# Nishad-Sharma/gpuRaytracer

Hardware: AMD Instinct MI355X
Metric: Msamples/sec (pixels×spp) Cornell box 1080p at 1/2/4/8 MI355X; HBM GB/s (higher is better)
Workload: dtype f32; 1 GPU; cornell_1920x1080_256spp_b3; width=1920, height=1080, spp_per_gpu=256, spp_frame=256, bounces=3, parallelism=single GPU

## Files before the change

gpuraytracer_amd/_native.py:

```python
from __future__ import annotations

import ctypes
import os

ABI_VERSION = 11
_HERE = os.path.dirname(os.path.abspath(__file__))
library_path = os.environ.get("RTPT_LIB") or os.path.join(_HERE, "librtpt.so")


class float3(ctypes.Structure):

    _fields_ = [("x", ctypes.c_float), ("y", ctypes.c_float), ("z", ctypes.c_float),
                ("_pad", ctypes.c_float)]

    def __iter__(self):
        return iter((self.x, self.y, self.z))


class float4(ctypes.Structure):
    _fields_ = [("x", ctypes.c_float), ("y", ctypes.c_float), ("z", ctypes.c_float),
                ("w", ctypes.c_float)]


class int2(ctypes.Structure):
# ... 235 lines not shown
                                               ctypes.POINTER(MaterialGPU),
                                               ctypes.POINTER(float3),
                                               ctypes.POINTER(SquareLightGPU),
                                               ctypes.POINTER(ctypes.c_uint32),
                                               ctypes.POINTER(SphereGPU)]),
    "rt_render_mis": (ctypes.c_int, [_P, ctypes.POINTER(MisParamsC), _P, _P]),
    "rt_scene_cornell_box_mis": (ctypes.c_int, [ctypes.c_int32, ctypes.c_int32,
                                                ctypes.POINTER(CameraGPU),
                                                ctypes.POINTER(MaterialGPU),
                                                ctypes.POINTER(float3),
                                                ctypes.POINTER(SquareLightGPU),
                                                ctypes.POINTER(ctypes.c_uint32)]),
    "rt_tonemap_rgba8": (None, [_P, ctypes.c_size_t, _P]),
    "rt_scene_describe": (ctypes.c_int, [ctypes.POINTER(SceneDesc), ctypes.POINTER(SceneInfo)]),
    "rt_scene_describe_ex": (ctypes.c_int, [ctypes.POINTER(SceneDesc), ctypes.POINTER(CreateOptions),
                                            ctypes.POINTER(SceneInfo)]),
    "rt_debug_camera_candidates": (ctypes.c_int, [ctypes.POINTER(SceneDesc)] + [ctypes.c_int32] * 4 + [_P]),
    "rt_debug_shadow_candidates": (ctypes.c_int, [ctypes.POINTER(SceneDesc)] + [ctypes.c_int32] * 4 +
                                   [_P, ctypes.POINTER(ctypes.c_int32)]),
    "rt_debug_cluster_kinds": (ctypes.c_int, [ctypes.POINTER(SceneDesc), ctypes.POINTER(ctypes.c_uint32),
                                              ctypes.c_uint32, ctypes.POINTER(ctypes.c_uint32)]),
    "rt_debug_light_mask": (ctypes.c_int, [ctypes.POINTER(SceneDesc), ctypes.POINTER(ctypes.c_uint64), _P,
                                           ctypes.c_uint32]),
}


class RtError(RuntimeError):

    def __init__(self, status: int, message: str):
        super().__init__(f"{STATUS.get(status, status)}: {message}")
        self.status = status


def _preload_hip_runtime():
    if os.environ.get("RTPT_SYSTEM_HIP") == "1":
        return
    import importlib.util
    spec = importlib.util.find_spec("torch")
    if spec is None or not spec.submodule_search_locations:
        return
    for d in spec.submodule_search_locations:
        cand = os.path.join(d, "lib", "libamdhip64.so")
        if os.path.exists(cand):
            ctypes.CDLL(cand, mode=ctypes.RTLD_GLOBAL)
            return

# ... 31 lines not shown
```

gpuraytracer_amd/csrc/rt_api.cpp:

```cpp
#include <rccl/rccl.h>

#include <stdio.h>
#include <stdlib.h>
#include <string.h>

#include <chrono>
#include <new>
#include <vector>

#include "rt_api_internal.hpp"

using namespace rtapi;

namespace {

class DevBuf {
public:
    DevBuf() = default;
    DevBuf(DevBuf&& o) noexcept : p_(o.p_), bytes_(o.bytes_) { o.p_ = nullptr; o.bytes_ = 0; }
    DevBuf& operator=(DevBuf&& o) noexcept {
        std::swap(p_, o.p_);
        std::swap(bytes_, o.bytes_);
        return *this;
    }
// ... 45 lines not shown
    kTriIsect, kTriShade, kPairIsect, kClusters, kSphLds, kSphLdsId,
    kSphBox,
    kSphIsect, kSphShade, kSphNodes, kSphPerm, kMisShade, kSceneArrays
};

}

struct rt_ctx {
    int device = 0;
    Stream stream;
    Event ev0, ev1;
    Event ev_u0, ev_u1;
    Event ev_tiles;
    rt::CompiledScene scene;
    DevBuf d_scene[kSceneArrays];
    DevBuf d_tri_nodes;
    uint32_t tri_build = kDefaultTriBuild;
    DevBuf d_tri_sorted, d_tri_perm;
    DevBuf d_refit;
    uint32_t tri_bvh_nodes = 0;
    rt::SceneTables tab{};
    bool sph_compact = false;
    uint64_t light_mask = 0;
    uint32_t tri_bvh_build_used = 0;
    uint32_t tri_leaf_max = 1;
    float tri_bvh_build_ms = 0.0f;
    size_t tri_bvh_temp_bytes = 0;
    float scene_compile_ms = 0.0f;
    DevBuf d_mis_tab;
    uint32_t mis_tab_S = 0;
    DevBuf d_mis_part;
    DevBuf d_out, d_out8;
    DevBuf d_rays, d_hits;
    DevBuf d_aov[3];
    DevBuf d_den[6];
    DevBuf d_seeds;
    bool seeds_ready = false;
    uint32_t seed_max = 0xFFFFFFFFu;
    DevBuf d_sum;
    bool sum_valid = false;
    uint32_t sum_row_start = 0, sum_row_step = 0, sum_row_count = 0;
    uint32_t sum_first = 0, sum_samples = 0;
    bool timed = false;
    rt::LaunchInfo launch{};
    bool launched = false;
    ncclComm_t comm = nullptr;
// ... 269 lines not shown
    const uint64_t total = (uint64_t)(p->accumulate ? c->sum_samples : 0u) + p->spp;
    if (total == 0 || total > 0xFFFFFFFFull)
        return fail(c, RT_ERR_INVALID_ARG, "samples in the sum must be in [1, 2^32)");

    const size_t pixels = (size_t)count * (size_t)c->scene.cam.W;
    int st;
    if ((st = check_out_format(c, p->flags)) != RT_OK) return st;
    const size_t out_bytes = pixels * pixel_bytes(p->flags);
    if (sums) {
        if (c->d_sum.bytes() < pixels * sizeof(float4)) c->sum_valid = false;
        if ((st = reserve(c, c->d_sum, pixels * sizeof(float4), "hipMalloc(sum)")) != RT_OK) return st;
    }
    void* kout = want_out ? out : nullptr;
    if (want_out && !out_is_device) {
        if ((st = reserve(c, c->d_out, out_bytes, "hipMalloc(out staging)")) != RT_OK) return st;
        kout = c->d_out.as<void>();
    }

    rt::KParams K;
    memset(&K, 0, sizeof(K));
    set_tables(&K, c->tab);
    K.tri_shade = c->d_scene[kTriShade].as<float4>();
    K.light_mask = c->light_mask;
    K.sph_lds = c->sph_compact ? c->d_scene[kSphLds].as<uint32_t>() : nullptr;
    K.sph_lds_id = c->d_scene[kSphLdsId].as<uint16_t>();
    K.sph_shade = c->d_scene[kSphShade].as<float4>();
    K.seeds = c->d_seeds.as<uint32_t>();
    K.sum = sums ? c->d_sum.as<float4>() : nullptr;
    K.out = kout;
    K.nE = c->scene.sph_lds_entries;
    set_camera(&K, c->scene.cam);
    memcpy(K.light_center, c->scene.light.center, sizeof(K.light_center));
    {
        uint32_t by, bz;
        memcpy(&by, &K.light_center[1], 4);
        memcpy(&bz, &K.light_center[2], 4);
        K.light_plain = (by != 0x80000000u && bz != 0x80000000u) ? 1u : 0u;
    }
    memcpy(K.light_color, c->scene.light.color, sizeof(K.light_color));
    K.spp = p->spp;
    K.sample_base = p->sample_base;
    K.row_start = start;
    K.row_step = step;
    K.row_count = count;
    K.accumulate = p->accumulate ? 1u : 0u;
    K.samples_total = (uint32_t)total;
// ... 413 lines not shown
    if (!compile_desc(d, ro.build, &c->scene, &err)) {
        delete c;
        return fail(nullptr, RT_ERR_INVALID_ARG, err);
    }
    c->scene_compile_ms = std::chrono::duration<float, std::milli>(clk::now() - t_compile).count();
    int status = RT_OK;
    std::string msg;
    do {
        if ((e = hipStreamCreateWithFlags(&c->stream.h, hipStreamNonBlocking)) != hipSuccess) {
            status = RT_ERR_NO_DEVICE; msg = std::string("hipStreamCreate: ") + hipGetErrorString(e); break;
        }
        if ((e = hipEventCreate(&c->ev0.h)) != hipSuccess || (e = hipEventCreate(&c->ev1.h)) != hipSuccess ||
            (e = hipEventCreateWithFlags(&c->ev_tiles.h, hipEventDisableTiming)) != hipSuccess) {
            status = RT_ERR_NO_DEVICE; msg = std::string("hipEventCreate: ") + hipGetErrorString(e); break;
        }
        if ((e = upload_scene(c)) != hipSuccess) {
            status = RT_ERR_OUT_OF_MEMORY; msg = std::string("scene upload: ") + hipGetErrorString(e); break;
        }
        if (needs_tri_bvh(c) && (status = build_tri_bvh(c, &msg)) != RT_OK) break;
        const size_t npx = (size_t)c->scene.cam.W * (size_t)c->scene.cam.H;
        if ((e = c->d_seeds.reserve(npx * sizeof(uint32_t))) != hipSuccess) {
            status = RT_ERR_OUT_OF_MEMORY; msg = std::string("hipMalloc(seeds): ") + hipGetErrorString(e); break;
        }
    } while (0);
    if (status != RT_OK) {
        delete c;
        return fail(nullptr, status, msg);
    }
    finish_scene(c);
    *out_ctx = c;
    return RT_OK;
}

int rt_destroy(rt_ctx* c) {
    if (!c) return RT_OK;
    DeviceGuard g(c->device);
    delete c;
    return RT_OK;
}

int rt_update_scene(rt_ctx* c, const rt_scene_desc* d, uint32_t flags) {
    static_assert(sizeof(rt_update_stats) == 32, "rt_update_stats layout");
    if (!c) return fail(nullptr, RT_ERR_INVALID_ARG, "ctx is null");
    if (!d) return fail(c, RT_ERR_INVALID_ARG, "rt_update_scene: scene is null");
    if (!d->camera) return fail(c, RT_ERR_INVALID_ARG, "rt_update_scene: camera is null");
    if (!d->square_lights || d->n_square_lights < 1)
// ... 251 lines not shown
int rt_debug_tri_bvh(const rt_ctx* c, rt_tri_bvh_dump* dump) {
    if (!c || !dump) return fail(nullptr, RT_ERR_INVALID_ARG, "null argument");
    if (!c->broken.empty()) return fail(const_cast<rt_ctx*>(c), RT_ERR_STATE, c->broken);
    if (!c->tri_bvh_build_used || !c->d_tri_nodes) return RT_ERR_STATE;
    const size_t nT = c->scene.tri_isect.size(), nn = c->tri_bvh_nodes;
    dump->n_triangles = (uint32_t)nT;
    dump->nodes_per_layout = (uint32_t)nn;
    dump->leaf_max = c->tri_leaf_max;
    dump->margin = c->scene.margin;
    DeviceGuard g(c->device);
    const struct { void* dst; const DevBuf& src; size_t bytes; } copies[4] = {
        {dump->nodes, c->d_tri_nodes, rt::kTriCompactLayouts * nn * sizeof(uint4)},
        {dump->sorted, c->d_tri_sorted, nT * sizeof(rt::TriIsect)},
        {dump->perm, c->d_tri_perm, nT * sizeof(uint32_t)},
        {dump->isect, c->d_scene[kTriIsect], nT * sizeof(rt::TriIsect)}};
    for (const auto& cp : copies) {
        if (!cp.dst) continue;
        const hipError_t e = hipMemcpy(cp.dst, cp.src.as<void>(), cp.bytes, hipMemcpyDeviceToHost);
        if (e != hipSuccess) return RT_ERR_LAUNCH;
    }
    return RT_OK;
}

int rt_last_launch(const rt_ctx* c, rt_launch_info* info) {
    if (!c || !info) return fail(nullptr, RT_ERR_INVALID_ARG, "null argument");
    if (!c->launched) return RT_ERR_STATE;
    memset(info, 0, sizeof(*info));
    static_assert(sizeof(info->kernel) == sizeof(c->launch.kernel), "kernel name buffer");
    memcpy(info->kernel, c->launch.kernel, sizeof(info->kernel));
    info->kernel[sizeof(info->kernel) - 1] = 0;
    info->lanes_per_pixel = c->launch.lanes;
    info->halton_tables = c->launch.tables;
    info->small_index = c->launch.small;
    info->block_threads = c->launch.threads;
    info->grid_x = c->launch.grid_x;
    info->grid_y = c->launch.grid_y;
    info->lds_bytes = c->launch.lds;
    return RT_OK;
}

int rt_debug_stats(rt_ctx* c, uint64_t* out, int n) {
    if (!c || !out || n <= 0) return fail(c, RT_ERR_INVALID_ARG, "null argument");
    DeviceGuard g(c->device);
    hipError_t e = rt::read_debug_stats(reinterpret_cast<unsigned long long*>(out), n);
    if (e == hipErrorNotSupported) return fail(c, RT_ERR_STATE, "not an RT_STATS build");
    if (e != hipSuccess) return hip_fail(c, RT_ERR_LAUNCH, "read stats", e);
// ... 10 lines not shown
```

gpuraytracer_amd/csrc/rt_api_host.cpp:

```cpp
#include <string.h>

#include <thread>
#include <vector>

#include "rt_api_internal.hpp"
#include "rt_beam.hpp"
#include "rt_mathcheck.hpp"
#include "rt_shaft.hpp"

namespace rtapi {

bool resolve_options(const rt_create_options* o, Resolved* r, const char** why) {
    *r = Resolved();
    if (!o) return true;
    for (uint32_t v : o->reserved)
        if (v != 0) { *why = "rt_create_options.reserved must be zero"; return false; }
    switch (o->scene_layout) {
        case RT_LAYOUT_AUTO: r->mem = rt::SceneMem::kAuto; break;
        case RT_LAYOUT_PAIRS: r->mem = rt::SceneMem::kPairLds; break;
        case RT_LAYOUT_SINGLE: r->mem = rt::SceneMem::kLdsSingle; break;
        case RT_LAYOUT_GLOBAL: r->mem = rt::SceneMem::kSmem; break;
        case RT_LAYOUT_PAIRS_SMEM: r->mem = rt::SceneMem::kPairSmem; break;
        case RT_LAYOUT_SORTED: r->mem = rt::SceneMem::kPairSorted; break;
        case RT_LAYOUT_BVH: r->mem = rt::SceneMem::kTriBvh; break;
        default: *why = "rt_create_options.scene_layout out of range"; return false;
    }
    if (o->lanes_per_pixel != 0 && o->lanes_per_pixel != 1 && o->lanes_per_pixel != 4 &&
        o->lanes_per_pixel != 16) {
        *why = "rt_create_options.lanes_per_pixel must be 0, 1, 4 or 16";
// ... 278 lines not shown
int rt_debug_cluster_kinds(const rt_scene_desc* d, uint32_t* flags, uint32_t capacity, uint32_t* n_clusters) {
    if (!desc_ok(d) || !n_clusters || (!flags && capacity)) return fail(nullptr, RT_ERR_INVALID_ARG, "null argument");
    rt::CompiledScene s;
    const char* err = nullptr;
    if (!compile_desc(d, rt::BuildOptions(), &s, &err)) return fail(nullptr, RT_ERR_INVALID_ARG, err);
    const size_t rec = 4 * rt::kCluF4, nC = s.clusters.size() / rec;
    *n_clusters = (uint32_t)nC;
    for (size_t c = 0; c < nC && c < capacity; ++c) memcpy(&flags[c], &s.clusters[c * rec + 15], 4);
    return RT_OK;
}

int rt_debug_light_mask(const rt_scene_desc* d, uint64_t* mask, float* records, uint32_t capacity_triangles) {
    if (!desc_ok(d) || !mask || (!records && capacity_triangles))
        return fail(nullptr, RT_ERR_INVALID_ARG, "null argument");
    rt::CompiledScene s;
    const char* err = nullptr;
    if (!compile_desc(d, rt::BuildOptions(), &s, &err)) return fail(nullptr, RT_ERR_INVALID_ARG, err);
    *mask = rt::light_mask(s);
    for (size_t k = 0; k < s.tri_shade.size() && k < capacity_triangles; ++k)
        memcpy(records + 16 * k, s.tri_shade[k].s, sizeof(s.tri_shade[k].s));
    return RT_OK;
}

int rt_debug_tri_bvh_host(const rt_scene_desc* d, const rt_create_options* opt, rt_tri_bvh_dump* dump) {
    if (!desc_ok(d) || !dump) return fail(nullptr, RT_ERR_INVALID_ARG, "null argument");
    Resolved ro;
    const char* why = nullptr;
    if (!resolve_options(opt, &ro, &why)) return fail(nullptr, RT_ERR_INVALID_ARG, why);
    rt::CompiledScene s;
    const char* err = nullptr;
    if (!compile_desc(d, ro.build, &s, &err)) return fail(nullptr, RT_ERR_INVALID_ARG, err);
    const size_t nT = s.tri_isect.size();
    dump->n_triangles = (uint32_t)nT;
    dump->nodes_per_layout = 0;
    dump->leaf_max = tri_leaf_clamp(ro.tri_leaf_max);
    dump->margin = s.margin;
    if (nT == 0) return fail(nullptr, RT_ERR_INVALID_ARG, "the scene has no triangles");
    if (dump->isect) memcpy(dump->isect, s.tri_isect.data(), nT * sizeof(rt::TriIsect));
    if (!dump->nodes && !dump->sorted && !dump->perm) return RT_OK;
    HostTree t;
    if (!rt::build_tri_sah(s.tri_isect, s.margin, &t.nodes, &t.sorted, &t.perm, ro.tri_leaf_max, ro.tri_leaf_cost))
        return fail(nullptr, RT_ERR_INVALID_ARG, "triangle BVH build: too many triangles (2^24)");
    dump_host_tree(t, dump);
    return RT_OK;
}

// ... 155 lines not shown
```

gpuraytracer_amd/csrc/rt_halton.hpp:

```cpp
#pragma once
#include <hip/hip_runtime.h>

#include "rt_kernel.hpp"

namespace rt {
namespace {

constexpr uint32_t kPrimes[24] = RT_PRIMES_INIT;

template <uint32_t D>
__device__ __forceinline__ float halton(uint32_t i) {
    static_assert(D < 24, "Halton dimension outside primes[]");
    constexpr uint32_t b = kPrimes[D];
    constexpr float invB = 1.0f / (float)b;
    float f = 1.0f;
    float r = 0.0f;
    while (i > 0) {
        f = f * invB;
        r = r + f * (float)(i % b);
        i = i / b;
    }
    return r;
}

// ... 39 lines not shown
#pragma unroll
        for (int k = 0; k < nd; ++k) {
            f = f * invB;
            float digit;
            x = digit_step<b>(x, digit);
            r = r + f * digit;
        }
        return r;
    }
}

constexpr int kTabDigits[24] = {0, 6, 4, 3, 2, 2, 0, 2, 2, 2, 2, 0, 0, 0, 0, 0, 0, 0, 0, 0, 0, 0, 0, 0};
constexpr uint32_t ipow(uint32_t b, int k) { return k == 0 ? 1u : b * ipow(b, k - 1); }
constexpr uint32_t tab_size(int D) { return kTabDigits[D] ? ipow(kPrimes[D], kTabDigits[D]) : 0u; }
constexpr uint32_t tab_offset(int D) { return D == 0 ? 0u : tab_offset(D - 1) + tab_size(D - 1); }
constexpr uint32_t kHaltonTabFloats = tab_offset(24);
constexpr float f_after(uint32_t b, int k) {
    float f = 1.0f;
    for (int j = 0; j < k; ++j) f = f * (1.0f / (float)b);
    return f;
}

template <uint32_t D>
__device__ __forceinline__ void fill_halton_table(float* tab, uint32_t tid, uint32_t nthreads) {
    constexpr uint32_t b = kPrimes[D];
    constexpr int k = kTabDigits[D];
    constexpr float invB = 1.0f / (float)b;
    constexpr uint32_t off = tab_offset(D), size = tab_size(D);
    for (uint32_t v0 = tid; v0 < size; v0 += nthreads) {
        uint32_t v = v0;
        float f = 1.0f;
        float r = 0.0f;
#pragma unroll
        for (int j = 0; j < k; ++j) {
            f = f * invB;
            r = r + f * (float)(v % b);
            v = v / b;
        }
        tab[off + v0] = r;
    }
}

__device__ __forceinline__ void fill_halton_tables(float* tab, uint32_t tid, uint32_t nthreads) {
    fill_halton_table<1>(tab, tid, nthreads);
    fill_halton_table<2>(tab, tid, nthreads);
    fill_halton_table<3>(tab, tid, nthreads);
    fill_halton_table<4>(tab, tid, nthreads);
    fill_halton_table<5>(tab, tid, nthreads);
    fill_halton_table<7>(tab, tid, nthreads);
    fill_halton_table<8>(tab, tid, nthreads);
    fill_halton_table<9>(tab, tid, nthreads);
    fill_halton_table<10>(tab, tid, nthreads);
    static_assert(kHaltonTabFloats == 729 + 625 + 343 + 121 + 169 + 361 + 529 + 841 + 961,
                  "table list");
}

template <uint32_t D>
__device__ __forceinline__ float halton_tab(uint32_t i, const float* tab) {
    constexpr uint32_t b = kPrimes[D];
    constexpr int k = kTabDigits[D];
    constexpr int nd = halton_digits(b, kSmallIndexMax);
    constexpr float invB = 1.0f / (float)b;
    constexpr uint32_t bk = ipow(b, k), off = tab_offset(D);
    static_assert(k > 0 && k < nd, "dimension without a table");
    float low;
    float x = digit_step<bk>((float)i, low);
    float r = tab[off + (uint32_t)low];
    constexpr float fk = f_after(b, k);
    float f = fk;
#pragma unroll
    for (int j = k; j < nd; ++j) {
        f = f * invB;
        float digit;
        x = digit_step<b>(x, digit);
        r = r + f * digit;
    }
    return r;
// ... 13 lines not shown
```

gpuraytracer_amd/csrc/rt_kernel.hip:

```cpp
#include <hip/hip_runtime.h>
#include <hip/hip_fp16.h>

#include <stddef.h>
#include <stdio.h>
#ifdef RT_LDS_CHECK
#include <hsa/hsa.h>
#endif

#include "rt_kernel.hpp"
#include "rt_halton.hpp"
#include "rt_beam.hpp"
#include "rt_shaft.hpp"
#include "rt_pixel.hpp"
#include "rt_trace.hpp"

namespace rt {

#ifdef RT_LDS_CHECK
__device__ uint32_t g_lds_overflow;
__device__ __forceinline__ bool lds_short(size_t end) {
    const uint32_t grp = ((const uint32_t*)__builtin_amdgcn_dispatch_ptr())[7];
    const size_t dyn = grp - __builtin_amdgcn_groupstaticsize();
    if (end <= dyn) return false;
    if (threadIdx.x == 0) atomicMax(&g_lds_overflow, (uint32_t)end);
// ... 423 lines not shown
#define RT_TRI_WAVES 8
#endif
__global__ __launch_bounds__(block_threads(GEO),
                             SPH ? kMinWavesPerEuSph
                                 : (GEO == kGeoPairClu ? kMinWavesPerEuClu
                                                       : (GEO == kGeoTriBvh ? RT_TRI_WAVES : kMinWavesPerEu)))
void path_trace_kernel(KParams P) {
    constexpr uint32_t NT = block_threads(GEO), WR = waves_per_row(GEO), WC = waves_per_col(GEO);
    extern __shared__ float4 lds[];
    SceneView sv;
    const SceneTables T = tables_of(P);
    if (geo_staged(GEO)) {
        const StagedF4<uint32_t> n = staged_f4(GEO, T.nT, T.nP, T.nC);
        RT_LDS_GUARD(16 * (size_t)(n.rec + n.clu) + (GEO == kGeoPairClu ? 4 * (size_t)kHaltonTabFloats : 0));
        stage_records<GEO, NT>(lds, T);
        if (GEO == kGeoSphLds) {
            __shared__ float sph_stash[GEO == kGeoSphLds ? 6 * kSphBlockThreads : 1];
            sv.xstash = sph_stash;
        }
        if (GEO == kGeoPairClu) {
            const uint32_t tab0 = n.rec + n.clu;
            const bool tab = halton_tables_on(GEO, SMALL, P.spp, L);
            sv.htab = tab ? reinterpret_cast<const float*>(lds + tab0) : nullptr;
            if (tab) fill_halton_tables(reinterpret_cast<float*>(lds + tab0), threadIdx.x, NT);
        }
        __syncthreads();
    }
    bind_scene<GEO, SPH>(sv, T, lds);

    const uint32_t kWX = (L == 1) ? 8u : P.wave_w, kWY = (64u / L) / kWX;
    uint32_t bx, by;
    xcd_tile(bx, by);
    auto pixel_of = [&](uint32_t t, uint32_t& x, uint32_t& j) {
        const uint32_t lane = t & 63u, wave = t >> 6, pix = lane / L;
        x = bx * (WR * kWX) + (wave % WR) * kWX + (pix % kWX);
        j = by * (WC * kWY) + (wave / WR) * kWY + (pix / kWX);
    };
    if constexpr (RT_CAM_CAND && GEO == kGeoPairClu) {
        if (sv.nP - 1u < 32u) {
            const uint32_t wave = wave_uniform(threadIdx.x >> 6);
            const uint32_t wx0 = bx * (WR * kWX) + (wave % WR) * kWX;
            const uint32_t wj0 = by * (WC * kWY) + (wave / WR) * kWY;
            const float y0 = (float)(P.row_start + wj0 * P.row_step);
            const float y1 = (float)(P.row_start + (wj0 + kWY - 1u) * P.row_step);
            const Beam beam = make_beam(ld_f3(P.cam_pos), ld_f3(P.cam_u), ld_f3(P.cam_v), ld_f3(P.cam_w), P.halfW,
                                        P.halfH, (float)P.W, (float)P.H, (float)wx0, (float)(wx0 + kWX - 1u), y0, y1);
            const uint32_t k = threadIdx.x & 63u;
// ... 40 lines not shown
    }
    __shared__ uint32_t seed_s[NT];
    __shared__ float lum_s[L > 1 ? 3 * (NT / L) : 1];
    f3 lum{0.0f, 0.0f, 0.0f};
    {
        const uint32_t t = threadIdx.x, sub = t % L;
        uint32_t x, j;
        pixel_of(t, x, j);
        const uint32_t y = P.row_start + j * P.row_step;
        seed_s[t] = P.seeds[(size_t)y * (size_t)P.W + x] + P.sample_base;
        if (P.accumulate) {
            const float4 prev = P.sum[(size_t)j * (size_t)P.W + x];
            lum = f3{prev.x, prev.y, prev.z};
        }
        const uint32_t slot = t / L;
        if (L > 1 && sub == 0) {
            lum_s[3 * slot] = lum.x;
            lum_s[3 * slot + 1] = lum.y;
            lum_s[3 * slot + 2] = lum.z;
        }
    }
    const f3 cu = ld_f3(P.cam_u), cv = ld_f3(P.cam_v), cw = ld_f3(P.cam_w);
    const float fW = (float)P.W, fH = (float)P.H;
    const uint32_t rounds = (P.spp + (L - 1)) / L;
    for (uint32_t r = 0; r < rounds; ++r) {
#ifdef RT_STATS
        const unsigned long long t_round = clock64();
#endif
        const uint32_t t = opaque_tid(), sub = t % L;
        const uint32_t n = (L == 1) ? r : min(r * L + sub, P.spp - 1u);
        PathState s;
        s.acc = f3{0.0f, 0.0f, 0.0f};
        {
            uint32_t x, j;
            pixel_of(t, x, j);
            const float fx = (float)x, fy = (float)(P.row_start + j * P.row_step);
            s.i = seed_s[t] + n;
            const float jx = halton_dim<0, SMALL>(s.i);
            const float jy = halton_dim<1, SMALL, GEO == kGeoPairClu>(s.i, sv.htab);
            s.d = camera_dir<GEO == kGeoTriBvh>(P, cu, cv, cw, fW, fH, fx, fy, jx, jy);
            s.o = ld_f3(P.cam_pos);
            s.thr = f3{1.0f, 1.0f, 1.0f};
#if RT_CENSUS == 1
            {
                const uint32_t i2 = cz(s.i);
                const float jx2 = halton_dim<0, SMALL>(i2);
                const float jy2 = halton_dim<1, SMALL, GEO == kGeoPairClu>(i2, sv.htab);
// ... 36 lines not shown
                f3 acc{lum_s[3 * slot], lum_s[3 * slot + 1], lum_s[3 * slot + 2]};
#pragma unroll
                for (int k = 0; k < L; ++k)
                    if (r * L + (uint32_t)k < P.spp) acc = acc + c[k];
                lum_s[3 * slot] = acc.x;
                lum_s[3 * slot + 1] = acc.y;
                lum_s[3 * slot + 2] = acc.z;
            }
        }
#ifdef RT_STATS
        if (!SPH && GEO != kGeoTriBvh) {
            RT_STAT(24, clock64() - t_round);
            RT_STAT(25, 1);
        }
#endif
    }
    uint32_t t = threadIdx.x;
    asm volatile("" : "+v"(t));
    if (L > 1) {
        if (t % L != 0) return;
        const uint32_t slot = t / L;
        lum = f3{lum_s[3 * slot], lum_s[3 * slot + 1], lum_s[3 * slot + 2]};
    }
    uint32_t x, j;
    pixel_of(t, x, j);
    const size_t o = (size_t)j * (size_t)P.W + x;
    if (P.sum) P.sum[o] = make_float4(lum.x, lum.y, lum.z, (float)P.samples_total);
    if (P.out) {
        const float fs = (float)P.samples_total;
        const float r = lum.x / fs, g = lum.y / fs, bl = lum.z / fs;
        store_pixel(P, o, r, g, bl);
    }
}

#include "rt_free.hpp"

#ifndef RT_SORTED_BVH_WAVES
#define RT_SORTED_BVH_WAVES 4
#endif
template <int B, int GEO, bool SPH, bool SMALL>
__global__ __launch_bounds__(kBlockThreads, GEO == kGeoPairLds ? kMinWavesPerEu : RT_SORTED_BVH_WAVES)
void path_trace_sorted_kernel(
    KParams P) {
    extern __shared__ float4 lds[];
    SceneView sv;
    const SceneTables T = tables_of(P);
// ... 42 lines not shown
__global__ void math_check_kernel(uint32_t lo, uint32_t n, unsigned long long* bad) {
    for (uint32_t i = blockIdx.x * blockDim.x + threadIdx.x; i < n; i += gridDim.x * blockDim.x) {
        const float x = __uint_as_float(lo + i);
        float y = x;
        asm volatile("" : "+v"(y));
        const float s = sqrt_cr(x), sr = sqrtf(y);
        const float r = rcp_cr(x), rr = 1.0f / y;
        const bool sbad = !(__float_as_uint(s) == __float_as_uint(sr) || (s != s && sr != sr));
        const bool rbad = !(__float_as_uint(r) == __float_as_uint(rr) || (r != r && rr != rr));
        if (sbad) atomicAdd(&bad[0], 1ull);
        if (rbad) atomicAdd(&bad[1], 1ull);
    }
}

__global__ void fill_seeds_kernel(uint32_t* seeds, uint64_t key, uint64_t n) {
    for (uint64_t p = (uint64_t)blockIdx.x * blockDim.x + threadIdx.x; p < n;
         p += (uint64_t)gridDim.x * blockDim.x) {
        uint64_t z = key + p + 0x9E3779B97F4A7C15ULL;
        z = (z ^ (z >> 30)) * 0xBF58476D1CE4E5B9ULL;
        z = (z ^ (z >> 27)) * 0x94D049BB133111EBULL;
        z = z ^ (z >> 31);
        seeds[p] = (uint32_t)(z & 0xFFFFFu);
    }
}

template <typename U>
__global__ void place_tiles_kernel(const U* __restrict__ gathered, U* __restrict__ frame, uint32_t row_u,
                                   size_t tile_u, uint32_t H, uint32_t N) {
    for (uint32_t y = blockIdx.y; y < H; y += gridDim.y) {
        const uint32_t k = y % N, j = y / N;
        const U* src = gathered + k * tile_u + (size_t)j * row_u;
        U* dst = frame + (size_t)y * row_u;
        for (uint32_t u = blockIdx.x * blockDim.x + threadIdx.x; u < row_u; u += gridDim.x * blockDim.x)
            dst[u] = src[u];
    }
}

hipError_t launch_place_tiles(const void* gathered, void* frame, size_t row_bytes, size_t tile_bytes,
                              uint32_t H, uint32_t N, hipStream_t stream) {
    if (H == 0 || N == 0 || row_bytes == 0) return hipSuccess;
    if (row_bytes % 4 || tile_bytes % 4) return hipErrorInvalidValue;
    const bool wide = row_bytes % 16 == 0 && tile_bytes % 16 == 0 &&
                      reinterpret_cast<uintptr_t>(gathered) % 16 == 0 && reinterpret_cast<uintptr_t>(frame) % 16 == 0;
    const size_t unit = wide ? 16 : 4;
    const uint32_t row_u = (uint32_t)(row_bytes / unit);
    const dim3 grid((row_u + 255u) / 256u, H < 65535u ? H : 65535u);
// ... 252 lines not shown
    const unsigned long long zero[40] = {0};
    return hipMemcpyToSymbol(HIP_SYMBOL(g_rt_stats), zero, sizeof(zero));
#else
    (void)out;
    (void)n;
    return hipErrorNotSupported;
#endif
}

hipError_t math_selfcheck(unsigned long long bad[2]) {
    unsigned long long* d = nullptr;
    hipError_t e = hipMalloc((void**)&d, 2 * sizeof(unsigned long long));
    if (e != hipSuccess) return e;
    if ((e = hipMemset(d, 0, 2 * sizeof(unsigned long long))) == hipSuccess) {
        hipLaunchKernelGGL(math_check_kernel, dim3(16384), dim3(256), 0, 0, 0u, 0x80000000u, d);
        hipLaunchKernelGGL(math_check_kernel, dim3(16384), dim3(256), 0, 0, 0x80000000u, 0x80000000u, d);
        if ((e = hipGetLastError()) == hipSuccess && (e = hipDeviceSynchronize()) == hipSuccess)
            e = hipMemcpy(bad, d, 2 * sizeof(unsigned long long), hipMemcpyDeviceToHost);
    }
    (void)hipFree(d);
    return e;
}

hipError_t launch_fill_seeds(uint32_t* seeds, uint64_t key, uint64_t n, hipStream_t stream) {
    if (n == 0) return hipSuccess;
    uint64_t blocks = (n + 255) / 256;
    if (blocks > 8192) blocks = 8192;
    hipLaunchKernelGGL(fill_seeds_kernel, dim3((unsigned)blocks), dim3(256), 0, stream, seeds,
                       key, n);
    return hipGetLastError();
}

}
```

gpuraytracer_amd/csrc/rt_kernel.hpp:

```cpp
#pragma once

#include <hip/hip_runtime.h>
#include <stddef.h>
#include <stdint.h>

#include "rt_math.h"
#include "rt_raydomain.h"

namespace rt {

constexpr uint32_t kBlockThreads = 256;
constexpr uint32_t kTile = 16;
constexpr size_t kMaxLdsBytes = 64 * 1024;
constexpr uint32_t kOutFp16 = 0x2u;
constexpr uint32_t kOutRgba8 = 0x10u;
constexpr uint32_t kPairF4 = 7;
constexpr uint32_t kSphBlockThreads = 64;
constexpr size_t kSphPairLdsMaxBytes = 6 * 1024;
constexpr uint32_t kCluF4 = 7;
#ifndef RT_CAM_CAND
#define RT_CAM_CAND 1
#endif
#ifndef RT_SHD_CAND
#define RT_SHD_CAND 1
#endif
#ifndef RT_CLU_ORDER
#define RT_CLU_ORDER 1
#endif
#ifndef RT_CLU_LEAN
#define RT_CLU_LEAN 1
#endif
constexpr uint32_t kTriCompactLayouts = 8;
constexpr uint32_t kTriBvhMinTriangles = 384;

struct SceneTables {
    const float4* tri_isect;
    const float4* pair_isect;
    const float4* clusters;
    const float4* sph_isect;
    const float4* sph_nodes;
    const uint32_t* sph_perm;
    const uint4* sph_box;
    const uint4* tri_nodes;
    const float4* tri_sorted;
    const uint32_t* tri_perm;
    uint32_t nT, nP, nS, nN;
    uint32_t nTN;
// ... 19 lines not shown
    void* out;
    uint32_t nT, nP, nS, nN;
    uint32_t nE;
    uint32_t nTN;
    float cam_pos[3], cam_u[3], cam_v[3], cam_w[3];
    float halfW, halfH;
    int32_t W, H;
    float light_center[3], light_color[3];
    uint32_t spp, sample_base;
    uint32_t row_start, row_step, row_count;
    uint32_t accumulate;
    uint32_t samples_total;
    uint32_t flags;
    uint32_t max_index;
    uint32_t lanes;
    uint32_t walk;
    uint32_t wave_w;
    uint32_t walk_leaf_den;
    uint32_t light_plain;
    const float4* clusters;
    uint32_t nC;
    uint32_t pair_free;
    uint64_t light_mask;
};

size_t kernel_lds_bytes(uint32_t n_tri, uint32_t n_pairs, uint32_t n_sph, uint32_t n_nodes);

enum KernelLayout : int {
    kLayTriLds = 0,
    kLayPairLds = 1,
    kLayTriGlobal = 2,
    kLayPairSorted = 3,
    kLayPairSmem = 4,
    kLayTriBvh = 5,
    kLayPairClu = 6,
    kLaySphLds = 7,
    kLayFreeSph = 8,
    kLayFreeTri = 9,
    kLaySortSph = 10,
    kLaySortTri = 11,
};
template <typename N>
struct StagedF4 {
    N rec, clu;
};
template <typename N = uint32_t>
// ... 117 lines not shown
};
hipError_t launch_denoise(const DenoiseParams& P, hipStream_t stream, LaunchInfo* info);

hipError_t launch_mis(const MisParams& P, SceneMem mem, hipStream_t stream);
size_t mis_lds_bytes(uint32_t n_tri, uint32_t n_pairs);
size_t mis_part_bytes(uint32_t camera_rays, size_t pixels);

hipError_t build_tri_lbvh(const float4* d_tri, uint32_t n, const float lo[3], const float hi[3],
                          float margin, uint4* d_nodes, float4* d_sorted, uint32_t* d_perm,
                          hipStream_t s);

hipError_t build_tri_gsah(const float4* d_tri, uint32_t n, float margin, uint32_t leaf_max, double trav_cost,
                          uint4* d_nodes, float4* d_sorted, uint32_t* d_perm, uint32_t* total_nodes,
                          size_t* temp_bytes, hipStream_t s);
hipError_t scan_u32(const uint32_t* in, uint32_t* out, uint32_t n, uint32_t* tile_sums, hipStream_t s);

size_t tri_refit_table_bytes(uint32_t total);
hipError_t refit_tri_bvh(const float4* d_tri, uint32_t n, float margin, uint4* d_nodes, uint32_t total,
                         float4* d_sorted, const uint32_t* d_perm, uint32_t** d_table, bool* table_made,
                         hipEvent_t ev0, hipEvent_t ev1, hipStream_t s);
hipError_t refit_format_errors(const uint32_t* d_table, uint32_t total, uint32_t* bad);

hipError_t launch_fill_seeds(uint32_t* seeds, uint64_t key, uint64_t n, hipStream_t stream);
hipError_t math_selfcheck(unsigned long long bad[2]);

hipError_t launch_place_tiles(const void* gathered, void* frame, size_t row_bytes, size_t tile_bytes,
                              uint32_t H, uint32_t N, hipStream_t stream);

}
```

gpuraytracer_amd/csrc/rt_trace.hpp:

```cpp
#pragma once
#include <hip/hip_runtime.h>

#include "rt_cluorder.hpp"
#include "rt_kernel.hpp"

namespace rt {
namespace {

__device__ __forceinline__ f3 ld_f3(const float* p) { return f3{p[0], p[1], p[2]}; }

__device__ __forceinline__ bool tri_test(const float4& A, const float4& Bq, const float4& C, f3 o,
                                         f3 d, float tmin, float tmax, float* t_out) {
    const f3 v0{A.x, A.y, A.z}, e1{A.w, Bq.x, Bq.y}, e2{Bq.z, Bq.w, C.x}, n{C.y, C.z, C.w};
    const f3 tv = o - v0;
    const f3 c = cross(tv, d);
    const float den = dot(n, d);
    const uint32_t sgn = __float_as_uint(den) & 0x80000000u;
    const uint32_t nsgn = sgn ^ 0x80000000u;
    const float bu = __uint_as_float(__float_as_uint(dot(e2, c)) ^ nsgn);
    const float bv = __uint_as_float(__float_as_uint(dot(e1, c)) ^ sgn);
    const float aden = fabsf(den);
    if (aden > 0.0f && bu >= 0.0f && bv >= 0.0f && bu + bv <= aden) {
        const float tn = __uint_as_float(__float_as_uint(dot(n, tv)) ^ nsgn);
        const float t = tn / aden;
// ... 763 lines not shown
            if (tri_test(sv.tri[3 * k], sv.tri[3 * k + 1], sv.tri[3 * k + 2], o, d, tmin, best,
                         &t)) {
                best = t;
                id = (int)k;
            }
        }
    }
    if (SPH && GEO == kGeoSphLds)
        sphere_walk_box<false>(sv.sbox, sv.sph, sv.sph_perm, sv.nSB, sv.nT, o, d, tmin, best, id);
    else if (SPH)
        sphere_closest(sv.node, sv.sph, sv.sph_perm, sv.nN, sv.nT, o, d, tmin, best, id);
    *t_io = best;
    return id;
}

template <int GEO, bool SPH, bool PACKET>
__device__ __forceinline__ bool any_hit(const SceneView& sv, f3& o, f3& d, float tmin, float tmax,
                                        f3 seg_lo, f3 seg_hi) {
    if (GEO == kGeoPairClu) {
        float tm = tmax;
        int id = -1;
        if (RT_SHD_CAND && RT_CAM_CAND && PACKET && sv.shd_avail) {
            if (sv.shd_mask == 0u) return false;
            cluster_query<true, true, true>(sv, o, d, tmin, &tm, &id);
        } else {
            cluster_query<true, true, false, false, RT_CLU_LEAN != 0>(sv, o, d, tmin, &tm, &id);
        }
        if (id >= 0) return true;
    } else if (geo_pairs(GEO)) {
        for (uint32_t k = 0; k < sv.nP; ++k) {
            const float4* r = sv.pair + kPairF4 * k;
            const float4 b0 = r[5], b1 = r[6];
            const bool overlap = seg_lo.x <= b0.w && seg_hi.x >= b0.x && seg_lo.y <= b1.x &&
                                 seg_hi.y >= b0.y && seg_lo.z <= b1.y && seg_hi.z >= b0.z;
            RT_STAT(8, 1);
            if (!__any(overlap)) continue;
            RT_STAT(9, 1);
            RT_STAT(10, __popcll(__ballot(1)));
            const float4 r0 = r[0], r1 = r[1], r2 = r[2], r3 = r[3], r4 = r[4];
            const PairDots q = pair_dots(r0, r1, r2, r3, r4, o, d);
            const bool pa = bary_ok(q.denA, q.a1, q.a2);
            const bool pb = bary_ok(q.denB, q.b1, q.b2);
            if (pa || pb) {
                RT_STAT(11, 1);
                const f3 nsel = pa ? f3{r2.y, r2.z, r2.w} : f3{r3.w, r4.x, r4.y};
                const float t = pair_t(nsel, q.tv, pa ? q.denA : q.denB);
// ... 93 lines not shown
```

include/rtpt.h:

```cpp
#ifndef RTPT_H
#define RTPT_H

#include "rt_types.h"

#ifdef __cplusplus
extern "C" {
#endif

#define RTPT_ABI_VERSION 11

#define RT_MAX_BOUNCES 4

typedef enum rt_status {
    RT_OK = 0,
    RT_ERR_INVALID_ARG = 1,
    RT_ERR_NO_DEVICE = 2,
    RT_ERR_OUT_OF_MEMORY = 3,
    RT_ERR_LAUNCH = 4,
    RT_ERR_STATE = 5,
    RT_ERR_COMM = 6
} rt_status;

typedef struct rt_ctx rt_ctx;

// ... 301 lines not shown
    uint32_t n_triangles;
    uint32_t n_triangle_pairs;
    uint32_t n_spheres;
    uint32_t lds_bytes;
    uint32_t n_sphere_nodes;
    uint32_t n_triangle_bvh_nodes;
    uint32_t n_box_clusters;
    uint32_t pair_free_mask;
    uint32_t sphere_kernel_lds_bytes;
    uint32_t kernel_layout;
    uint32_t kernel_lds_bytes;
} rt_scene_info;
int rt_scene_describe(const rt_scene_desc* scene, rt_scene_info* info);
int rt_scene_describe_ex(const rt_scene_desc* scene, const rt_create_options* opt, rt_scene_info* info);

int rt_debug_camera_candidates(const rt_scene_desc* scene, int32_t x0, int32_t x1, int32_t y0, int32_t y1,
                               uint8_t* may_hit);

int rt_debug_shadow_candidates(const rt_scene_desc* scene, int32_t x0, int32_t x1, int32_t y0, int32_t y1,
                               uint8_t* may_occlude, int32_t* available);

int rt_debug_cluster_kinds(const rt_scene_desc* scene, uint32_t* flags, uint32_t capacity, uint32_t* n_clusters);

int rt_debug_light_mask(const rt_scene_desc* scene, uint64_t* mask, float* records, uint32_t capacity_triangles);

void rt_tonemap_rgba8(const float* rgba32f, size_t n_pixels, uint8_t* rgba8);

#ifdef __cplusplus
}
#endif

#endif
```

Baseline: 28860 Msamples/s.

## Precompute Halton tables once, skip dead camera tiles, shortcut small shadow masks

Halton radical-inverse tables are now built once per context by a small kernel and copied into LDS with float4 loads at block start, instead of being recomputed in every block. Blocks whose camera-candidate mask is empty skip all sample rounds and write zero radiance. Shadow any-hit queries with only a few candidate pairs test those pairs directly rather than running the full cluster query. This reduces per-block setup and traversal overhead, but adds a global-memory read per block and a separate code path that must stay consistent with the full query.

```diff
diff --git a/gpuraytracer_amd/_native.py b/gpuraytracer_amd/_native.py
--- a/gpuraytracer_amd/_native.py
+++ b/gpuraytracer_amd/_native.py
@@ -281,6 +281,8 @@
                                               ctypes.c_uint32, ctypes.POINTER(ctypes.c_uint32)]),
     "rt_debug_light_mask": (ctypes.c_int, [ctypes.POINTER(SceneDesc), ctypes.POINTER(ctypes.c_uint64), _P,
                                            ctypes.c_uint32]),
+    "rt_debug_halton_table": (ctypes.c_int, [_P, ctypes.c_uint32, ctypes.POINTER(ctypes.c_uint32), _P, _P]),
+    "rt_debug_halton_table_device": (ctypes.c_int, [_P, _P, ctypes.c_uint32]),
 }
 
 
diff --git a/gpuraytracer_amd/csrc/rt_api.cpp b/gpuraytracer_amd/csrc/rt_api.cpp
--- a/gpuraytracer_amd/csrc/rt_api.cpp
+++ b/gpuraytracer_amd/csrc/rt_api.cpp
@@ -91,6 +91,7 @@
     rt::SceneTables tab{};
     bool sph_compact = false;
     uint64_t light_mask = 0;
+    DevBuf d_halton_tab;
     uint32_t tri_bvh_build_used = 0;
     uint32_t tri_leaf_max = 1;
     float tri_bvh_build_ms = 0.0f;
@@ -406,6 +407,7 @@
     set_tables(&K, c->tab);
     K.tri_shade = c->d_scene[kTriShade].as<float4>();
     K.light_mask = c->light_mask;
+    K.halton_tab = c->d_halton_tab.as<float>();
     K.sph_lds = c->sph_compact ? c->d_scene[kSphLds].as<uint32_t>() : nullptr;
     K.sph_lds_id = c->d_scene[kSphLdsId].as<uint16_t>();
     K.sph_shade = c->d_scene[kSphShade].as<float4>();
@@ -865,6 +867,13 @@
         if ((e = c->d_seeds.reserve(npx * sizeof(uint32_t))) != hipSuccess) {
             status = RT_ERR_OUT_OF_MEMORY; msg = std::string("hipMalloc(seeds): ") + hipGetErrorString(e); break;
         }
+        if ((e = c->d_halton_tab.resize_exact(sizeof(float) * rt::kHaltonTabLdsFloats)) != hipSuccess) {
+            status = RT_ERR_OUT_OF_MEMORY; msg = std::string("hipMalloc(halton tables): ") + hipGetErrorString(e); break;
+        }
+        if ((e = rt::launch_fill_halton_tables(c->d_halton_tab.as<float>(), c->stream)) != hipSuccess ||
+            (e = hipStreamSynchronize(c->stream)) != hipSuccess) {
+            status = RT_ERR_LAUNCH; msg = std::string("halton tables: ") + hipGetErrorString(e); break;
+        }
     } while (0);
     if (status != RT_OK) {
         delete c;
@@ -1162,6 +1171,17 @@
     return RT_OK;
 }
 
+int rt_debug_halton_table_device(const rt_ctx* c, float* table, uint32_t capacity) {
+    if (!c || !table) return fail(nullptr, RT_ERR_INVALID_ARG, "null argument");
+    if (capacity < rt::kHaltonTabLdsFloats)
+        return fail(const_cast<rt_ctx*>(c), RT_ERR_INVALID_ARG, "rt_debug_halton_table_device: capacity below the table's size");
+    if (!c->d_halton_tab) return RT_ERR_STATE;
+    DeviceGuard g(c->device);
+    const hipError_t e =
+        hipMemcpy(table, c->d_halton_tab.as<void>(), sizeof(float) * rt::kHaltonTabLdsFloats, hipMemcpyDeviceToHost);
+    return e == hipSuccess ? RT_OK : RT_ERR_LAUNCH;
+}
+
 int rt_last_launch(const rt_ctx* c, rt_launch_info* info) {
     if (!c || !info) return fail(nullptr, RT_ERR_INVALID_ARG, "null argument");
     if (!c->launched) return RT_ERR_STATE;
diff --git a/gpuraytracer_amd/csrc/rt_api_host.cpp b/gpuraytracer_amd/csrc/rt_api_host.cpp
--- a/gpuraytracer_amd/csrc/rt_api_host.cpp
+++ b/gpuraytracer_amd/csrc/rt_api_host.cpp
@@ -5,6 +5,7 @@
 
 #include "rt_api_internal.hpp"
 #include "rt_beam.hpp"
+#include "rt_halton.hpp"
 #include "rt_mathcheck.hpp"
 #include "rt_shaft.hpp"
 
@@ -329,6 +330,21 @@
     return RT_OK;
 }
 
+int rt_debug_halton_table(float* table, uint32_t capacity, uint32_t* n_floats, uint32_t* offsets, uint32_t* sizes) {
+    static_assert(rt::kHaltonTabFloats == rt::kHaltonTabLdsFloats, "rt_kernel.hpp's size of the tables");
+    if (!n_floats || (!table && capacity)) return fail(nullptr, RT_ERR_INVALID_ARG, "null argument");
+    *n_floats = rt::kHaltonTabFloats;
+    for (int D = 0; D < 24; ++D) {
+        if (offsets) offsets[D] = rt::tab_offset(D);
+        if (sizes) sizes[D] = rt::tab_size(D);
+    }
+    if (!table) return RT_OK;
+    if (capacity < rt::kHaltonTabFloats)
+        return fail(nullptr, RT_ERR_INVALID_ARG, "rt_debug_halton_table: capacity below the table's size");
+    rt::fill_halton_tables(table, 0u, 1u);
+    return RT_OK;
+}
+
 int rt_debug_tri_bvh_host(const rt_scene_desc* d, const rt_create_options* opt, rt_tri_bvh_dump* dump) {
     if (!desc_ok(d) || !dump) return fail(nullptr, RT_ERR_INVALID_ARG, "null argument");
     Resolved ro;
diff --git a/gpuraytracer_amd/csrc/rt_halton.hpp b/gpuraytracer_amd/csrc/rt_halton.hpp
--- a/gpuraytracer_amd/csrc/rt_halton.hpp
+++ b/gpuraytracer_amd/csrc/rt_halton.hpp
@@ -85,7 +85,7 @@
 }
 
 template <uint32_t D>
-__device__ __forceinline__ void fill_halton_table(float* tab, uint32_t tid, uint32_t nthreads) {
+RT_HD void fill_halton_table(float* tab, uint32_t tid, uint32_t nthreads) {
     constexpr uint32_t b = kPrimes[D];
     constexpr int k = kTabDigits[D];
     constexpr float invB = 1.0f / (float)b;
@@ -104,7 +104,7 @@
     }
 }
 
-__device__ __forceinline__ void fill_halton_tables(float* tab, uint32_t tid, uint32_t nthreads) {
+RT_HD void fill_halton_tables(float* tab, uint32_t tid, uint32_t nthreads) {
     fill_halton_table<1>(tab, tid, nthreads);
     fill_halton_table<2>(tab, tid, nthreads);
     fill_halton_table<3>(tab, tid, nthreads);
@@ -116,6 +116,21 @@
     fill_halton_table<10>(tab, tid, nthreads);
     static_assert(kHaltonTabFloats == 729 + 625 + 343 + 121 + 169 + 361 + 529 + 841 + 961,
                   "table list");
+}
+
+template <uint32_t NT>
+__device__ __forceinline__ void copy_halton_tables(float* tab, const float* __restrict__ src, uint32_t tid) {
+    constexpr uint32_t n4 = kHaltonTabFloats / 4u, tail = kHaltonTabFloats % 4u;
+    constexpr uint32_t rounds = (n4 + NT - 1u) / NT;
+    const float4* s4 = reinterpret_cast<const float4*>(src);
+    float4* d4 = reinterpret_cast<float4*>(tab);
+    float4 v[rounds];
+#pragma unroll
+    for (uint32_t k = 0; k < rounds; ++k) v[k] = s4[tid + k * NT < n4 ? tid + k * NT : n4 - 1u];
+#pragma unroll
+    for (uint32_t k = 0; k < rounds; ++k)
+        if (tid + k * NT < n4) d4[tid + k * NT] = v[k];
+    if (tid < tail) tab[4u * n4 + tid] = src[4u * n4 + tid];
 }
 
 template <uint32_t D>
diff --git a/gpuraytracer_amd/csrc/rt_kernel.hip b/gpuraytracer_amd/csrc/rt_kernel.hip
--- a/gpuraytracer_amd/csrc/rt_kernel.hip
+++ b/gpuraytracer_amd/csrc/rt_kernel.hip
@@ -469,7 +469,7 @@
             const uint32_t tab0 = n.rec + n.clu;
             const bool tab = halton_tables_on(GEO, SMALL, P.spp, L);
             sv.htab = tab ? reinterpret_cast<const float*>(lds + tab0) : nullptr;
-            if (tab) fill_halton_tables(reinterpret_cast<float*>(lds + tab0), threadIdx.x, NT);
+            if (tab) copy_halton_tables<NT>(reinterpret_cast<float*>(lds + tab0), P.halton_tab, threadIdx.x);
         }
         __syncthreads();
     }
@@ -556,7 +556,13 @@
     }
     const f3 cu = ld_f3(P.cam_u), cv = ld_f3(P.cam_v), cw = ld_f3(P.cam_w);
     const float fW = (float)P.W, fH = (float)P.H;
-    const uint32_t rounds = (P.spp + (L - 1)) / L;
+    uint32_t rounds = (P.spp + (L - 1)) / L;
+    constexpr bool kDeadSkip = RT_CAM_CAND && RT_DEAD_SKIP && GEO == kGeoPairClu && !SPH;
+    bool dead = false;
+    if constexpr (kDeadSkip) {
+        dead = sv.cam_avail && sv.cam_mask == 0u;
+        if (dead) rounds = 0u;
+    }
     for (uint32_t r = 0; r < rounds; ++r) {
 #ifdef RT_STATS
         const unsigned long long t_round = clock64();
@@ -639,6 +645,9 @@
         const uint32_t slot = t / L;
         lum = f3{lum_s[3 * slot], lum_s[3 * slot + 1], lum_s[3 * slot + 2]};
     }
+    if constexpr (kDeadSkip) {
+        if (dead && P.spp != 0u) lum = lum + f3{0.0f, 0.0f, 0.0f};
+    }
     uint32_t x, j;
     pixel_of(t, x, j);
     const size_t o = (size_t)j * (size_t)P.W + x;
@@ -727,6 +736,10 @@
         z = z ^ (z >> 31);
         seeds[p] = (uint32_t)(z & 0xFFFFFu);
     }
+}
+
+__global__ __launch_bounds__(kBlockThreads) void halton_tables_kernel(float* tab) {
+    fill_halton_tables(tab, threadIdx.x, kBlockThreads);
 }
 
 template <typename U>
@@ -1025,6 +1038,11 @@
     return e;
 }
 
+hipError_t launch_fill_halton_tables(float* tab, hipStream_t stream) {
+    hipLaunchKernelGGL(halton_tables_kernel, dim3(1), dim3(kBlockThreads), 0, stream, tab);
+    return hipGetLastError();
+}
+
 hipError_t launch_fill_seeds(uint32_t* seeds, uint64_t key, uint64_t n, hipStream_t stream) {
     if (n == 0) return hipSuccess;
     uint64_t blocks = (n + 255) / 256;
diff --git a/gpuraytracer_amd/csrc/rt_kernel.hpp b/gpuraytracer_amd/csrc/rt_kernel.hpp
--- a/gpuraytracer_amd/csrc/rt_kernel.hpp
+++ b/gpuraytracer_amd/csrc/rt_kernel.hpp
@@ -23,6 +23,12 @@
 #endif
 #ifndef RT_SHD_CAND
 #define RT_SHD_CAND 1
+#endif
+#ifndef RT_SHD_SHORT
+#define RT_SHD_SHORT 3
+#endif
+#ifndef RT_DEAD_SKIP
+#define RT_DEAD_SKIP 1
 #endif
 #ifndef RT_CLU_ORDER
 #define RT_CLU_ORDER 1
@@ -88,6 +94,7 @@
     uint32_t nC;
     uint32_t pair_free;
     uint64_t light_mask;
+    const float* halton_tab;
 };
 
 size_t kernel_lds_bytes(uint32_t n_tri, uint32_t n_pairs, uint32_t n_sph, uint32_t n_nodes);
@@ -251,6 +258,7 @@
 hipError_t refit_format_errors(const uint32_t* d_table, uint32_t total, uint32_t* bad);
 
 hipError_t launch_fill_seeds(uint32_t* seeds, uint64_t key, uint64_t n, hipStream_t stream);
+hipError_t launch_fill_halton_tables(float* tab, hipStream_t stream);
 hipError_t math_selfcheck(unsigned long long bad[2]);
 
 hipError_t launch_place_tiles(const void* gathered, void* frame, size_t row_bytes, size_t tile_bytes,
diff --git a/gpuraytracer_amd/csrc/rt_trace.hpp b/gpuraytracer_amd/csrc/rt_trace.hpp
--- a/gpuraytracer_amd/csrc/rt_trace.hpp
+++ b/gpuraytracer_amd/csrc/rt_trace.hpp
@@ -809,6 +809,13 @@
         int id = -1;
         if (RT_SHD_CAND && RT_CAM_CAND && PACKET && sv.shd_avail) {
             if (sv.shd_mask == 0u) return false;
+            if (RT_SHD_SHORT > 0 && __builtin_popcount(sv.shd_mask) <= RT_SHD_SHORT) {
+                for (uint32_t m = sv.shd_mask; m != 0u && id < 0; m &= m - 1u) {
+                    const uint32_t k = (uint32_t)__builtin_ctz(m);
+                    pair_test_rank<true>(sv.pair + kPairF4 * k, k, o, d, tmin, &tm, &id);
+                }
+                return id >= 0;
+            }
             cluster_query<true, true, true>(sv, o, d, tmin, &tm, &id);
         } else {
             cluster_query<true, true, false, false, RT_CLU_LEAN != 0>(sv, o, d, tmin, &tm, &id);
diff --git a/include/rtpt.h b/include/rtpt.h
--- a/include/rtpt.h
+++ b/include/rtpt.h
@@ -347,6 +347,9 @@
 
 int rt_debug_cluster_kinds(const rt_scene_desc* scene, uint32_t* flags, uint32_t capacity, uint32_t* n_clusters);
 
+int rt_debug_halton_table(float* table, uint32_t capacity, uint32_t* n_floats, uint32_t* offsets, uint32_t* sizes);
+int rt_debug_halton_table_device(const rt_ctx* ctx, float* table, uint32_t capacity);
+
 int rt_debug_light_mask(const rt_scene_desc* scene, uint64_t* mask, float* records, uint32_t capacity_triangles);
 
 void rt_tonemap_rgba8(const float* rgba32f, size_t n_pixels, uint8_t* rgba8);
```

New measurement: 29320 Msamples/s, median of 6. 1.6% higher.
